# yuanhao-chen-nyoeghau/Wav2Vec2ForBrain

Measured on AMD Instinct MI355X. Metric: train steps/sec + CTC loss, b2p2t_gru+w2v bs=32 seq=1024, higher is better.
Workload: dtype bf16; 1 GPU; b2p2t_gru+w2v wav2vec2-base (12L/768), GRU H256x2 bidir, train mode, unfreeze=brain_encoder, Adam; global_batch=32, per_gpu_batch=32, seq_len=1024, parallelism=dp1

## Files before the change

### include/b2p_hip.h

```cpp
#ifndef B2P_HIP_H
#define B2P_HIP_H
#include <stdint.h>

#ifdef __cplusplus
extern "C" {
#endif

typedef void* b2p_stream_t;

const char* b2p_last_error(void);
int b2p_version(void);
int b2p_abi_sizes(int64_t* out3);
int b2p_timing_enable(int family, int max_events);
int b2p_timing_read(int family, float* total_ms, int* count, double* total_flops);

typedef struct {
  const void* ptr;
  int64_t ld;
  int64_t bs1, bs2;
  const int64_t* gather1;
  int32_t inner_is_k;
  int32_t conv;
  int32_t conv_T_out, conv_T_in, conv_stride, conv_pad, conv_Cg;
  int32_t dtype;
// ... 96 lines not shown
                      float* workspace, b2p_stream_t stream);
int b2p_layernorm_fwd16(const float* x, const float* gamma, const float* beta, float* y, uint16_t* y16,
                        float* mean, float* rstd, int64_t rows, int64_t cols, float eps,
                        float drop_p, uint64_t drop_seed, b2p_stream_t stream);
int b2p_layernorm_bwd16(const float* dy, const float* x, const float* gamma, const float* mean,
                        const float* rstd, float* dx, float* dgamma, float* dbeta, int64_t rows,
                        int64_t cols, const float* dx_accum, float drop_p, uint64_t drop_seed,
                        float* dx_dropped, float in_drop_p, uint64_t in_drop_seed, float* dbias_in,
                        uint16_t* d16, float* workspace, b2p_stream_t stream);
int b2p_layernorm_bwd_acc2(const float* dy, const float* x, const float* gamma, const float* mean,
                           const float* rstd, float* dx, float* dgamma, float* dbeta, int64_t rows,
                           int64_t cols, const float* dx_accum, const float* dx_accum2, float drop_p,
                           uint64_t drop_seed, float* dx_dropped, float in_drop_p, uint64_t in_drop_seed,
                           float* dbias_in, uint16_t* d16, float* workspace, b2p_stream_t stream);
int b2p_layernorm_fwd16_sel(const float* x, const float* gamma, const float* beta, float* y, uint16_t* y16,
                            float* mean, float* rstd, int64_t rows, int64_t cols, float eps, float drop_p,
                            uint64_t drop_seed, const int32_t* gate, const float* skip, const uint16_t* skip16,
                            b2p_stream_t stream);
int b2p_layernorm_fwd_x16_sel(const float* x, const float* gamma, const float* beta, float* y, uint16_t* y16,
                              int y16_fp16, uint16_t* y16b, float* mean, float* rstd, int64_t rows, int64_t cols,
                              float eps, const int32_t* gate, const float* skip, const uint16_t* skip16,
                              const uint16_t* skip16b, b2p_stream_t stream);
int b2p_layernorm_bwd_gated(const float* dy, const float* x, const float* gamma, const float* mean,
                            const float* rstd, float* dx, float* dgamma, float* dbeta, int64_t rows,
                            int64_t cols, const float* dx_accum, const float* dx_accum2, float drop_p,
                            uint64_t drop_seed, float* dx_dropped, float in_drop_p, uint64_t in_drop_seed,
                            float* dbias_in, uint16_t* d16, const int32_t* dy_gate, const int32_t* acc2_gate,
                            float* workspace, b2p_stream_t stream);
#define B2P_LNB_IN_DROP 1u
int b2p_layernorm_bwd_flags(const float* dy, const float* x, const float* gamma, const float* mean,
                            const float* rstd, float* dx, float* dgamma, float* dbeta, int64_t rows,
                            int64_t cols, const float* dx_accum, const float* dx_accum2, float drop_p,
                            uint64_t drop_seed, float* dx_dropped, float in_drop_p, uint64_t in_drop_seed,
                            float* dbias_in, uint16_t* d16, const int32_t* dy_gate, const int32_t* acc2_gate,
                            uint32_t flags, float* workspace, b2p_stream_t stream);

int b2p_cast_bf16(const float* x, uint16_t* y, int64_t n, b2p_stream_t stream);
int b2p_cast16_2d(const float* x, int64_t R, int64_t C, int64_t ldx, uint16_t* y, int64_t ldy, int fp16,
                  b2p_stream_t stream);
int b2p_transpose_bf16(const float* x, uint16_t* y, int64_t R, int64_t C, int64_t ldy, int64_t col0,
                       b2p_stream_t stream);

int b2p_softmax_fwd(const float* S, float* P, float* Pd, int64_t rows, int64_t n, int64_t ld,
                    float drop_p, uint64_t drop_seed, b2p_stream_t stream);
int b2p_softmax_bwd(const float* P, const float* dPd, float* dS, int64_t rows, int64_t n,
                    int64_t ld, float drop_p, uint64_t drop_seed, b2p_stream_t stream);

int b2p_act_fwd(const float* pre, float* out, int64_t n, int act, b2p_stream_t stream);
int b2p_act_bwd(const float* dy, const float* pre, float* dx, int64_t n, int act,
                b2p_stream_t stream);

int b2p_gauss_smooth(const float* x, const float* taps, int ntaps, float* y, int64_t B,
                     int64_t L, int64_t C, b2p_stream_t stream);
int b2p_unfold_col2im(const float* dA, const float* Z, float* dX, int64_t B, int64_t L,
                      int64_t C, int64_t T, int ktaps, int stride, b2p_stream_t stream);
int b2p_day_reduce(const float* per_sample, const int64_t* day_idx, int64_t B, int64_t ndays,
                   int64_t elems, float* out, b2p_stream_t stream);

int b2p_unfold16(const float* x, uint16_t* U, int64_t B, int64_t L, int64_t C, int64_t k,
                 int64_t stride, b2p_stream_t stream);
int b2p_unfold_weight16(const float* w0, const float* w1, int64_t G, int64_t C, int64_t k, int64_t stride,
                        uint16_t* wf, int fp16, uint16_t* wb, b2p_stream_t stream);
int b2p_pad_rows16(const float* src, uint16_t* dst, int64_t B, int64_t T, int64_t N, int64_t R, int64_t lead,
                   b2p_stream_t stream);
int b2p_cast16_tail(const float* x, uint16_t* y, int64_t n, int64_t n_total, int fp16, b2p_stream_t stream);
int b2p_gather_recs(const int64_t* recs, int nrec, b2p_stream_t stream);
int b2p_conv_weight_permute(const float* in, float* out, int64_t O, int64_t I, int64_t ntaps,
                            int inverse, b2p_stream_t stream);
int b2p_conv_weight_transpose_flip(const float* w, float* out, int64_t G, int64_t Og, int64_t I,
                                   int64_t ntaps, b2p_stream_t stream);

int b2p_ctc_greedy_wer(const float* logits, int64_t B, int64_t T, int64_t C, const int64_t* target, int64_t S,
                       int blank, int eos, int delim, int32_t* out_tokens, int32_t* out_ntok, int32_t* errs,
                       int32_t* nwords, b2p_stream_t stream);
int b2p_ctc_greedy_cer(const float* logits, int64_t B, int64_t T, int64_t C, const int64_t* target, int64_t S,
                       int blank, int eos, int delim, const uint8_t* tok_chars, const int32_t* tok_len,
                       int32_t* char_errs, int32_t* nchars, b2p_stream_t stream);
int64_t b2p_ctc_beam_workspace(int64_t B, int64_t T, int64_t beam);
int b2p_ctc_prefix_beam(const float* logits, int64_t B, int64_t T, int64_t C, const int32_t* lens, int64_t beam,
                        int blank, float token_min_logp, float beam_prune_logp, int32_t* workspace,
                        int32_t* out_tokens, int32_t* out_len, float* out_score, b2p_stream_t stream);
typedef struct {
  const uint64_t* trie_keys;
  const int32_t* trie_child;
  const int32_t* node_word;
  const uint64_t* ng_keys;
  const float* ng_vals;
  int64_t trie_capacity, ng_capacity;
  uint64_t trie_seed, ng_seed;
  int32_t order, unk_id, bos_id, eos_id;
  float beta;
  int32_t reserved;
} b2p_ngram_lm;
int64_t b2p_ctc_beam_lm_workspace(int64_t B, int64_t T, int64_t beam);
int b2p_ctc_prefix_beam_lm(const float* logits, int64_t B, int64_t T, int64_t C, const int32_t* lens, int64_t beam,
                           int blank, int delim, float token_min_logp, float beam_prune_logp,
                           const b2p_ngram_lm* lm, float unk_score_offset, float unk_score_scaled,
                           int score_boundary, int32_t* workspace, int32_t* out_tokens, int32_t* out_len,
                           float* out_ctc_logp, float* out_score, b2p_stream_t stream);

int b2p_posconv16_fwd(const float* e, const uint16_t* w16, const float* bias, float* xsum, float* pre,
                      uint16_t* e16, int64_t B, int64_t T, int64_t D, int64_t groups, b2p_stream_t stream);
int b2p_posconv16_bwd_data(const float* dxsum, const float* pre, const uint16_t* wt16, float* de, uint16_t* dpre16,
                           float* colpart, int64_t B, int64_t T, int64_t D, int64_t groups, b2p_stream_t stream);
int b2p_posconv16_wgrad(const uint16_t* dpre16, const uint16_t* e16, float* dwp, int64_t B, int64_t T, int64_t D,
                        int64_t groups, b2p_stream_t stream);
// ... 189 lines not shown
```

### wav2vec2forbrain_amd/_lib.py

```python
from __future__ import annotations

import ctypes
import os

import torch

_HERE = os.path.dirname(os.path.abspath(__file__))
LIB_PATH = os.environ.get("B2P_LIB_PATH") or os.path.join(_HERE, "libb2p_hip.so")

c_i64 = ctypes.c_int64
c_i32 = ctypes.c_int32
c_f32 = ctypes.c_float
c_f64 = ctypes.c_double
c_u64 = ctypes.c_uint64
c_u32 = ctypes.c_uint32
c_p = ctypes.c_void_p


class Operand(ctypes.Structure):
    _fields_ = [
        ("ptr", c_p), ("ld", c_i64), ("bs1", c_i64), ("bs2", c_i64), ("gather1", c_p),
        ("inner_is_k", c_i32), ("conv", c_i32),
        ("conv_T_out", c_i32), ("conv_T_in", c_i32), ("conv_stride", c_i32), ("conv_pad", c_i32),
        ("conv_Cg", c_i32), ("dtype", c_i32), ("conv_sample_stride", c_i64),
# ... 14 lines not shown
class GemmDesc(ctypes.Structure):
    _fields_ = [
        ("M", c_i64), ("N", c_i64), ("K", c_i64), ("nz1", c_i32), ("nz2", c_i32),
        ("A", Operand), ("B", Operand), ("ep", Epilogue),
        ("precision", c_i32), ("timing_family", c_i32), ("flops", c_f64),
        ("ksplit", c_i32), ("kchunk", c_i32), ("workspace", c_p), ("workspace_floats", c_i64),
    ]


class NgramLM(ctypes.Structure):
    _fields_ = [
        ("trie_keys", c_p), ("trie_child", c_p), ("node_word", c_p), ("ng_keys", c_p), ("ng_vals", c_p),
        ("trie_capacity", c_i64), ("ng_capacity", c_i64), ("trie_seed", c_u64), ("ng_seed", c_u64),
        ("order", c_i32), ("unk_id", c_i32), ("bos_id", c_i32), ("eos_id", c_i32), ("beta", c_f32),
        ("reserved", c_i32),
    ]


_SIGS = {
    "b2p_last_error": (ctypes.c_char_p, []),
    "b2p_version": (c_i32, []),
    "b2p_abi_sizes": (c_i32, [c_p]),
    "b2p_timing_enable": (c_i32, [c_i32, c_i32]),
    "b2p_timing_read": (c_i32, [c_i32, ctypes.POINTER(c_f32), ctypes.POINTER(c_i32), ctypes.POINTER(c_f64)]),
    "b2p_gemm": (c_i32, [ctypes.POINTER(GemmDesc), c_p]),
    "b2p_colsum_workspace": (c_i64, [c_i64, c_i64]),
    "b2p_colsum": (c_i32, [c_p, c_i64, c_i64, c_i64, c_p, c_i32, c_p, c_p]),
    "b2p_colsum_batched": (c_i32, [c_p, c_p, c_i64, c_i64, c_i64, c_i64, c_i64, c_i32, c_p, c_i32, c_p, c_p]),
    "b2p_colsum_parts": (c_i32, [c_p, c_i64, c_i64, c_p, c_i32, c_p]),
    "b2p_attn16_dkv_variant": (c_i32, [c_i32]),
    "b2p_set_gate_batch": (c_i32, [c_p]),
    "b2p_split3_bf16": (c_i32, [c_p, c_i64, c_i64, c_i64, c_p, c_i64, c_i32, c_i32, c_p]),
    "b2p_i64_fill": (c_i32, [c_p, ctypes.POINTER(c_i64), c_i32, c_p]),
    "b2p_colsum_pin_begin": (c_i32, []),
    "b2p_colsum_pin_end": (c_i64, []),
    "b2p_colsum_unpin": (c_i32, [c_i64]),
    "b2p_colsum_pool_state": (c_i64, [c_i64, ctypes.POINTER(c_i64)]),
    "b2p_dropout": (c_i32, [c_p, c_p, c_i64, c_f32, c_u64, c_p]),
    "b2p_layernorm_fwd": (c_i32, [c_p, c_p, c_p, c_p, c_p, c_p, c_i64, c_i64, c_f32, c_f32, c_u64, c_p]),
    "b2p_layernorm_bwd_workspace": (c_i64, [c_i64, c_i64]),
    "b2p_layernorm_bwd": (c_i32, [c_p, c_p, c_p, c_p, c_p, c_p, c_p, c_p, c_i64, c_i64, c_p, c_f32, c_u64,
                                  c_p, c_f32, c_u64, c_p, c_p, c_p]),
    "b2p_layernorm_fwd16": (c_i32, [c_p, c_p, c_p, c_p, c_p, c_p, c_p, c_i64, c_i64, c_f32, c_f32, c_u64, c_p]),
    "b2p_layernorm_bwd16": (c_i32, [c_p, c_p, c_p, c_p, c_p, c_p, c_p, c_p, c_i64, c_i64, c_p, c_f32, c_u64,
                                    c_p, c_f32, c_u64, c_p, c_p, c_p, c_p]),
    "b2p_layernorm_bwd_acc2": (c_i32, [c_p, c_p, c_p, c_p, c_p, c_p, c_p, c_p, c_i64, c_i64, c_p, c_p, c_f32, c_u64,
                                       c_p, c_f32, c_u64, c_p, c_p, c_p, c_p]),
    "b2p_cast_bf16": (c_i32, [c_p, c_p, c_i64, c_p]),
    "b2p_softmax_fwd": (c_i32, [c_p, c_p, c_p, c_i64, c_i64, c_i64, c_f32, c_u64, c_p]),
    "b2p_softmax_bwd": (c_i32, [c_p, c_p, c_p, c_i64, c_i64, c_i64, c_f32, c_u64, c_p]),
    "b2p_act_fwd": (c_i32, [c_p, c_p, c_i64, c_i32, c_p]),
    "b2p_act_bwd": (c_i32, [c_p, c_p, c_p, c_i64, c_i32, c_p]),
    "b2p_gauss_smooth": (c_i32, [c_p, c_p, c_i32, c_p, c_i64, c_i64, c_i64, c_p]),
    "b2p_unfold_col2im": (c_i32, [c_p, c_p, c_p, c_i64, c_i64, c_i64, c_i64, c_i32, c_i32, c_p]),
    "b2p_day_reduce": (c_i32, [c_p, c_p, c_i64, c_i64, c_i64, c_p, c_p]),
    "b2p_unfold16": (c_i32, [c_p, c_p, c_i64, c_i64, c_i64, c_i64, c_i64, c_p]),
    "b2p_unfold_weight16": (c_i32, [c_p, c_p, c_i64, c_i64, c_i64, c_i64, c_p, c_i32, c_p, c_p]),
    "b2p_pad_rows16": (c_i32, [c_p, c_p, c_i64, c_i64, c_i64, c_i64, c_i64, c_p]),
    "b2p_cast16_tail": (c_i32, [c_p, c_p, c_i64, c_i64, c_i32, c_p]),
    "b2p_gather_recs": (c_i32, [c_p, c_i32, c_p]),
    "b2p_conv_weight_permute": (c_i32, [c_p, c_p, c_i64, c_i64, c_i64, c_i32, c_p]),
    "b2p_conv_weight_transpose_flip": (c_i32, [c_p, c_p, c_i64, c_i64, c_i64, c_i64, c_p]),
    "b2p_weight_norm_workspace": (c_i64, [c_i64, c_i64, c_i64]),
    "b2p_weight_norm_fwd": (c_i32, [c_p, c_p, c_p, c_p, c_i64, c_i64, c_i64, c_p, c_p]),
    "b2p_weight_norm_bwd": (c_i32, [c_p, c_p, c_p, c_p, c_p, c_p, c_i64, c_i64, c_i64, c_p, c_p]),
    "b2p_gru_fwd": (c_i32, [c_p, c_p, c_p, c_p, c_p, c_p, c_i64, c_i64, c_i64, c_i32, c_p]),
    "b2p_gru_bwd": (c_i32, [c_p, c_p, c_p, c_p, c_p, c_p, c_p, c_p, c_p, c_i64, c_i64, c_i64, c_i32, c_p]),
    "b2p_gru16_supported": (c_i32, [c_i64]),
    "b2p_gru16_lane_floats": (c_i64, [c_i64, c_i64, c_i64, c_i32, c_i32]),
    "b2p_gru_lane_permute": (c_i32, [c_p, c_p, c_i64, c_i64, c_i64, c_i32, c_i32, c_i32, c_u32, c_i32, c_p]),
    "b2p_gru_fwd16": (c_i32, [c_p, c_p, c_p, c_p, c_p, c_p, c_i64, c_i64, c_i64, c_i32, c_p]),
    "b2p_gru_bwd16": (c_i32, [c_p, c_p, c_p, c_p, c_p, c_p, c_p, c_i64, c_i64, c_i64, c_i32, c_p]),
    "b2p_gru_mc_supported": (c_i32, [c_i64]),
    "b2p_gru_mc_workspace": (c_i64, [c_i64, c_i64, c_i32]),
    "b2p_gru_fwd_mc": (c_i32, [c_p, c_p, c_p, c_p, c_p, c_p, c_p, c_i64, c_i64, c_i64, c_i32, c_p]),
    "b2p_gru_bwd_mc": (c_i32, [c_p, c_p, c_p, c_p, c_p, c_p, c_p, c_p, c_p, c_i64, c_i64, c_i64, c_i32, c_p]),
    "b2p_gru_mc_status": (c_i32, [c_p, c_p, c_i32, c_p]),
    "b2p_gru_mc_debug_withhold": (c_i32, [c_i32]),
    "b2p_gru32_supported": (c_i32, [c_i64]),
    "b2p_gru32_workspace": (c_i64, [c_i64, c_i64, c_i32]),
    "b2p_gru_fwd32": (c_i32, [c_p, c_p, c_p, c_p, c_p, c_p, c_p, c_i64, c_i64, c_i64, c_i32, c_p]),
    "b2p_gru_bwd32": (c_i32, [c_p, c_p, c_p, c_p, c_p, c_p, c_p, c_p, c_p, c_i64, c_i64, c_i64, c_i32, c_p]),
    "b2p_gru_hprev": (c_i32, [c_p, c_p, c_p, c_i64, c_i64, c_i64, c_i32, c_p]),
    "b2p_attn16_fwd": (c_i32, [c_p, c_p, c_p, c_i64, c_i64, c_i64, c_i64, c_f32, c_f32, c_u64, c_p, c_p]),
    "b2p_attn16_fwd_f16": (c_i32, [c_p, c_p, c_p, c_p, c_i64, c_i64, c_i64, c_i64, c_f32, c_f32, c_u64, c_p, c_p]),
    "b2p_attn16_fwd_keep": (c_i32, [c_p, c_p, c_p, c_i64, c_i64, c_i64, c_i64, c_f32, c_f32, c_p, c_p]),
    "b2p_attn16_fwd_f16_keep": (c_i32, [c_p, c_p, c_p, c_p, c_i64, c_i64, c_i64, c_i64, c_f32, c_f32, c_p, c_p]),
    "b2p_attn16_keep_masks": (c_i32, [c_p, c_p, c_i64, c_i64, c_i64, c_i64, c_f32, c_p]),
    "b2p_attn16_bwd": (c_i32, [c_p, c_p, c_p, c_p, c_p, c_p, c_i64, c_i64, c_i64, c_i64, c_f32, c_f32, c_u64, c_p,
                               c_p]),
    "b2p_attn16_bwd_f16": (c_i32, [c_p, c_p, c_p, c_p, c_p, c_p, c_i64, c_i64, c_i64, c_i64, c_f32, c_f32, c_u64, c_p,
                               c_p]),
    "b2p_attn32_supported": (c_i32, [c_i64, c_i64]),
    "b2p_attn32_fwd": (c_i32, [c_p, c_p, c_p, c_i64, c_i64, c_i64, c_i64, c_f32, c_f32, c_u64, c_p]),
    "b2p_attn32_bwd": (c_i32, [c_p, c_p, c_p, c_p, c_p, c_i64, c_i64, c_i64, c_i64, c_f32, c_f32, c_u64, c_p]),
    "b2p_attn32_long_supported": (c_i32, [c_i64, c_i64]),
    "b2p_attn32_long_fwd": (c_i32, [c_p, c_p, c_p, c_i64, c_i64, c_i64, c_i64, c_f32, c_f32, c_u64, c_p]),
    "b2p_attn32_long_bwd": (c_i32, [c_p, c_p, c_p, c_p, c_p, c_i64, c_i64, c_i64, c_i64, c_f32, c_f32, c_u64, c_p]),
    "b2p_ctc_workspace": (c_i64, [c_i64, c_i64, c_i64, c_i64]),
    "b2p_ctc_fwd_bwd": (c_i32, [c_p, c_p, c_p, c_p, c_i64, c_i64, c_i64, c_i64, c_i32, c_p, c_p, c_p, c_p, c_p]),
    "b2p_adam_multi": (c_i32, [c_p, c_i32, c_i64, c_f32, c_f32, c_f32, c_f32, c_f32, c_f32, c_f32, c_p]),
    "b2p_adam_multi_dev": (c_i32, [c_p, c_i32, c_i64, c_p, c_f32, c_f32, c_f32, c_f32, c_p, c_p, c_p]),
    "b2p_cast16_2d": (c_i32, [c_p, c_i64, c_i64, c_i64, c_p, c_i64, c_i32, c_p]),
    "b2p_accum_recs": (c_i32, [c_p, c_i32, c_p]),
    "b2p_accum_rows_recs": (c_i32, [c_p, c_i32, c_p]),
    "b2p_adam_recs": (c_i32, [c_p, c_i32, c_f32, c_f64, c_f64, c_f32, c_f32, c_f32, c_f32, c_p, c_p, c_p, c_p]),
# ... 114 lines not shown
```

### wav2vec2forbrain_amd/functional.py

```python
from __future__ import annotations

import collections
import contextlib
import functools
import ctypes
import math
import threading
import weakref

import os

import torch

from . import _lib
from ._lib import GemmDesc, Operand, Epilogue

ACT = {"none": 0, None: 0, "gelu": 1, "softsign": 2, "silu": 3, "swish": 3,
       "linear": 0, "gelu_python": 1,
       "gelu_new": 4, "gelu_fast": 4, "gelu_pytorch_tanh": 4, "gelu_accurate": 4,
       "gelu_10": 5, "quick_gelu": 6, "laplace": 7, "mish": 8, "relu": 9, "relu2": 10, "relu6": 11,
       "sigmoid": 12, "tanh": 13}
EPILOGUE_ACTS = frozenset({0, 1, 2, 3})
_ACT_NAME = {}
for _k, _v in ACT.items():
# ... 1174 lines not shown
def to16h(x):
    t = getattr(x, "_h16", None)
    if t is not None and t[0] == x._version:
        return t[1]
    xc = x.contiguous()
    out = torch.empty(xc.shape, device=x.device, dtype=torch.float16)
    _lib.call("b2p_cast16_2d", _p(xc), 1, xc.numel(), xc.numel(), _p(out), xc.numel(), 1, _st())
    return out


def _ln_fwd16(x2d, g, b, eps, drop_p=0.0, seed=0, sel=None):
    rows, cols = x2d.shape
    y = torch.empty_like(x2d)
    y16 = torch.empty(rows, cols, device=x2d.device, dtype=BF16)
    mean = torch.empty(rows, device=x2d.device)
    rstd = torch.empty(rows, device=x2d.device)
    if sel is not None:
        _lib.call("b2p_layernorm_fwd16_sel", _p(x2d), _p(g), _p(b), _p(y), _p(y16), _p(mean), _p(rstd), rows, cols,
                  float(eps), float(drop_p), seed, _p(sel[0]), _p(sel[1]), _p(sel[2]), _st())
        return y, y16, mean, rstd
    _lib.call("b2p_layernorm_fwd16", _p(x2d), _p(g), _p(b), _p(y), _p(y16), _p(mean), _p(rstd), rows, cols,
              float(eps), float(drop_p), seed, _st())
    return y, y16, mean, rstd


def _ln_bwd16(dy, x, g, mean, rstd, need_params=True, dx_accum=None, drop_p=0.0, seed=0, in_drop_p=-1.0,
              in_seed=0, dbias_in=None, dx_accum2=None, lazy=None, dy_gate=None, acc2_gate=None, want_dxd=True):
    rows, cols = x.shape
    lz = _ln_lazy(lazy, need_params, dbias_in)
    dx = torch.empty_like(x)
    dg = torch.empty(cols, device=x.device) if need_params and not lz else None
    db = torch.empty(cols, device=x.device) if need_params and not lz else None
    ws = torch.empty(int(_lib.load().b2p_layernorm_bwd_workspace(rows, cols)), device=x.device)
    dxd = torch.empty_like(x) if in_drop_p >= 0.0 and want_dxd else None
    d16 = torch.empty(rows, cols, device=x.device, dtype=BF16)
    if in_drop_p >= 0.0 and not want_dxd:
        _lib.call("b2p_layernorm_bwd_flags", _p(dy), _p(x), _p(g), _p(mean), _p(rstd), _p(dx), _p(dg), _p(db), rows,
                  cols, _p(dx_accum), _p(dx_accum2), float(drop_p), seed, None, float(in_drop_p), in_seed,
                  None if lz else _p(dbias_in), _p(d16), _p(dy_gate), _p(acc2_gate), _lib.LNB_IN_DROP, _p(ws), _st())
    elif dy_gate is not None or acc2_gate is not None:
        _lib.call("b2p_layernorm_bwd_gated", _p(dy), _p(x), _p(g), _p(mean), _p(rstd), _p(dx), _p(dg), _p(db), rows,
                  cols, _p(dx_accum), _p(dx_accum2), float(drop_p), seed, _p(dxd), float(max(in_drop_p, 0.0)),
                  in_seed, None if lz else _p(dbias_in), _p(d16), _p(dy_gate), _p(acc2_gate), _p(ws), _st())
    else:
        _lib.call("b2p_layernorm_bwd_acc2", _p(dy), _p(x), _p(g), _p(mean), _p(rstd), _p(dx), _p(dg), _p(db), rows,
                  cols, _p(dx_accum), _p(dx_accum2), float(drop_p), seed, _p(dxd), float(max(in_drop_p, 0.0)),
                  in_seed, None if lz else _p(dbias_in), _p(d16), _p(ws), _st())
    if lz:
        dg, db = _ln_parts(ws, rows, cols, 0), _ln_parts(ws, rows, cols, 1)
        dbias_in = _ln_parts(ws, rows, cols, 2) if dbias_in is not None else None
    return (dx, dg, db, dxd, d16) if lazy is None else (dx, dg, db, dxd, d16, dbias_in)


@_prec_follow
class _FrontEnd(torch.autograd.Function):
    @staticmethod
    def forward(ctx, x, day_idxs, day_weights, day_bias, taps):
        _chk(x, "front_end.x")
        _chk(day_weights, "front_end.day_weights")
        B, L, C = x.shape
        xs = torch.empty_like(x)
        _lib.call("b2p_gauss_smooth", _p(x), _p(taps), taps.numel(), _p(xs), B, L, C, _st())
        z = torch.empty_like(x)
        s = torch.empty_like(x)
        gemm(L, C, C, op(xs, 0, C, True, bs1=L * C), op(day_weights, 0, C, False, bs1=C * C, gather=day_idxs),
             s, C, cbs1=L * C, nz1=B, bias=day_bias, biasbs1=C, bias_gather=day_idxs, pre_out=z,
             act=ACT["softsign"])
        ctx.save_for_backward(xs, z, day_idxs, day_weights)
        ctx.n_days = day_weights.shape[0]
        return s

    @staticmethod
    def backward(ctx, ds):
        xs, z, day_idxs, day_weights = ctx.saved_tensors
        ds = ds.contiguous()
        B, L, C = xs.shape
        dz = _act_bwd(ds, z, ACT["softsign"])
        dW = dbias = None
        if ctx.needs_input_grad[2]:
            per = torch.empty(B, C, C, device=xs.device)
            gemm(C, C, L, op(xs, 0, C, False, bs1=L * C), op(dz, 0, C, False, bs1=L * C), per, C, cbs1=C * C, nz1=B)
            dW = torch.empty_like(day_weights)
            _lib.call("b2p_day_reduce", _p(per), _p(day_idxs), B, ctx.n_days, C * C, _p(dW), _st())
        if ctx.needs_input_grad[3]:
            per_b = torch.empty(B, C, device=xs.device)
            colsum_batched(dz, B, L, C, per_b)
            dbias = torch.empty(ctx.n_days, 1, C, device=xs.device)
            _lib.call("b2p_day_reduce", _p(per_b), _p(day_idxs), B, ctx.n_days, C, _p(dbias), _st())
        return None, None, dW, dbias, None


def front_end(x, day_idxs, day_weights, day_bias, taps):
    with _fp32_if("front"):
        return _FrontEnd.apply(x.contiguous(), day_idxs.to(torch.int64).contiguous(), day_weights, day_bias, taps)


class Unfolded:

    def __init__(self, src: torch.Tensor, kernel: int, stride: int):
        self.src = src
        self.kernel = kernel
        self.stride = stride
        B, L, C = src.shape
        self.T = (L - kernel) // stride + 1
        self.shape = (B, self.T, C * kernel)

    def materialize(self) -> torch.Tensor:
        B, L, C = self.src.shape
        idx = torch.arange(self.T, device=self.src.device)[:, None] * self.stride + torch.arange(self.kernel, device=self.src.device)[None, :]
        win = self.src[:, idx, :]
        return win.permute(0, 1, 3, 2).reshape(B, self.T, C * self.kernel)


_GRUMC = [True]
_GRUMC_BWD = [None]
_GRU32 = [True]
GRU32_MODES = (3,)
_GRU32_NARROW_MAX = 512


@contextlib.contextmanager
def persistent_gru32(on: bool = True):
    old = _GRU32[0]
    _GRU32[0] = bool(on)
    try:
        yield
    finally:
        _GRU32[0] = old


def _gru_recurrence(H: int) -> str:
    lib = _lib.load()
    fast = bf16_mode() or (_state.prec == 3 and "grurec1" in (_state.x3forms or ()))
    if fast and lib.b2p_gru16_supported(H):
        return "gru16"
    if fast and _GRUMC[0] and lib.b2p_gru_mc_supported(H):
        return "mc"
    if not fast and _state.prec in GRU32_MODES and _GRU32[0] and lib.b2p_gru32_supported(H):
        if H <= _GRU32_NARROW_MAX or "gru32w" in (_state.x3forms or ()):
            return "gru32"
    return "step"


def _gru_recurrence_bwd(fwd: str, H: int) -> str:
    if fwd == "gru16" or _GRUMC_BWD[0] is None:
        return fwd
    if _GRUMC_BWD[0] and _lib.load().b2p_gru_mc_supported(H):
# ... 132 lines not shown

class _UnfoldProj:

    @staticmethod
    def forward(x, wih, bias_cat, gi, s, need_dx):
        B, T, IN, G3, N3, L, C = s.B, s.T, s.IN, s.G3, s.N3, s.L, s.C
        wperm = torch.empty(N3, IN, device=s.dev)
        for d in range(s.ndir):
            _lib.call("b2p_conv_weight_permute", _p(wih[d]), _p(wperm, d * G3 * IN), G3, C, s.ktaps, 0, _st())
        U16 = None
        if bf16_mode() and not _state.fwd16:
            U16 = torch.empty(B * T, IN, device=s.dev, dtype=BF16)
            _lib.call("b2p_unfold16", _p(x), _p(U16), B, L, C, s.ktaps, s.stride, _st())
            wperm = cast16(wperm)
            A = op(U16, 0, IN, True)
        else:
            A = conv_op(x, 0, C, T, L, s.stride, 0, IN, L * C, True)
            A.conv_Cg = C
        gemm(B * T, N3, IN, A, op(wperm, 0, IN, True), gi, N3, bias=bias_cat)
        return wperm, U16

    @staticmethod
    def backward(dgi, x, wih, kept, s, need_dx, need_dw):
        B, T, IN, N3, L, C = s.B, s.T, s.IN, s.N3, s.L, s.C
        wperm, U16 = kept
        dg = cast16(dgi) if U16 is not None else dgi
        dx, dws = None, [None] * s.ndir
        if any(need_dw):
            dwp = torch.empty(N3, IN, device=s.dev)
            U = op(U16, 0, IN, False) if U16 is not None else conv_op(x, 0, C, T, L, s.stride, 0, C, L * C, False)
            gemm(N3, IN, B * T, op(dg, 0, N3, False), U, dwp, IN)
            dws = _unfold_dw(dwp, s)
        if need_dx:
            dA = torch.empty(B * T, IN, device=s.dev)
            gemm(B * T, IN, N3, op(dg, 0, N3, True), op(wperm, 0, IN, False), dA, IN)
            dx = torch.empty(B, L, C, device=s.dev)
            _lib.call("b2p_unfold_col2im", _p(dA), None, _p(dx), B, L, C, T, s.ktaps, s.stride, _st())
        return dx, dws


class _ImplicitUnfoldProj:

    @staticmethod
    def forward(x, wih, bias_cat, gi, s, need_dx):
        B, T, IN, N3, L, C, ktaps, stride = s.B, s.T, s.IN, s.N3, s.L, s.C, s.ktaps, s.stride
        half = _state.fwd16
        wf = torch.empty(N3, IN, device=s.dev, dtype=torch.float16 if half else BF16)
        wperm = torch.empty((ktaps // stride) * N3, stride * C, device=s.dev, dtype=BF16) if need_dx else None
        _lib.call("b2p_unfold_weight16", _p(wih[0]), _p(wih[1]) if s.ndir == 2 else None, s.G3, C, ktaps, stride,
                  _p(wf), int(half), _p(wperm), _st())
        s16 = _ImplicitUnfoldProj.source16(x, s, half)
        gemm(T, N3, IN, op(s16, 0, stride * C, True, bs1=L * C), op(wf, 0, IN, True), gi, N3, cbs1=T * N3, nz1=B,
             bias=bias_cat)
        return wperm, (None if half else s16)

    @staticmethod
    def source16(x, s, half):
        n_s, tail = s.B * s.L * s.C, (s.ktaps - s.stride) * s.C
        s16 = torch.empty(n_s + tail, device=s.dev, dtype=torch.float16 if half else BF16)
        _lib.call("b2p_cast16_tail", _p(x), _p(s16), n_s, n_s + tail, int(half), _st())
        return s16

    @staticmethod
    def backward(dgi, x, wih, kept, s, need_dx, need_dw):
        B, IN, N3, L, C, ktaps, stride = s.B, s.IN, s.N3, s.L, s.C, s.ktaps, s.stride
        wperm, s16 = kept
        R, lead = L // stride, ktaps // stride - 1
        dgp = torch.empty((lead + B * R) * N3, device=s.dev, dtype=BF16)
        _lib.call("b2p_pad_rows16", _p(dgi), _p(dgp), B, s.T, N3, R, lead, _st())
        dx, dws = None, [None] * s.ndir
        if any(need_dw):
            s16 = s16 if s16 is not None else _ImplicitUnfoldProj.source16(x, s, False)
            dwp = torch.empty(N3, IN, device=s.dev)
            gemm(N3, IN, B * R, op(dgp, lead * N3, N3, False), op(s16, 0, stride * C, False), dwp, IN)
            del s16
            dws = _unfold_dw(dwp, s)
        if need_dx:
            dx = torch.empty(B, L, C, device=s.dev)
            gemm(B * R, stride * C, (ktaps // stride) * N3, op(dgp, 0, N3, True), op(wperm, 0, stride * C, False),
                 dx, stride * C)
        return dx, dws


@_prec_follow
class _GRULayer(torch.autograd.Function):
    @staticmethod
    def forward(ctx, x, unf_meta, H, ndir, h0, *weights):
        dev, G3 = x.device, 3 * H
        if unf_meta is not None:
            ktaps, stride = unf_meta
            B, L, C = x.shape
            s = _GRUShape(B, (L - ktaps) // stride + 1, C * ktaps, H, G3, ndir * G3, ndir, dev, L, C, ktaps, stride)
        else:
            s = _GRUShape(*x.shape, H, G3, ndir * G3, ndir, dev, None, None, None, None)
        B, T = s.B, s.T
        wih, whh, bih, bhh = ([weights[4 * d + i] for d in range(ndir)] for i in range(4))
        for w in wih + whh:
            _chk(w, "gru.weight")
        gi = torch.empty(B, T, ndir * G3, device=dev)
        rec = _gru_recurrence(H)
        fold = rec == "gru16" and bhh[0] is not None
        whh_s = torch.empty(ndir, G3, H, device=dev)
        bhh_s = torch.empty(ndir, G3, device=dev) if bhh[0] is not None else None
        bias_cat = torch.empty(ndir * G3, device=dev) if (any(b is not None for b in bih) or fold) else None
        recs = []
        for d in range(ndir):
            recs += [_p(whh_s, d * G3 * H), _p(whh[d]), 0, G3 * H]
            if bhh_s is not None:
                recs += [_p(bhh_s, d * G3), _p(bhh[d]), 0, G3]
            if bias_cat is not None:
# ... 1811 lines not shown
```

### wav2vec2forbrain_amd/model/b2p2t_model.py

```python
from __future__ import annotations

import math
from typing import Literal, cast

import torch
from pydantic import BaseModel
from torch import nn

from .. import functional as Fn
from ..datasets.batch_types import B2tSampleBatch
from .b2tmodel import B2TModel, ModelOutput

DEFAULT_UNFOLDER_KERNEL_LEN = 32


class B2P2TModelArgsModel(BaseModel):
    input_layer_nonlinearity: Literal["softsign"] = "softsign"
    unfolder_kernel_len: int = DEFAULT_UNFOLDER_KERNEL_LEN
    unfolder_stride_len: int = 4
    gaussian_smooth_width: float = 0.3


class GaussianSmoothing(nn.Module):

    def __init__(self, channels, kernel_size: int, sigma: float, dim=1):
        super().__init__()
        if dim != 1:
            raise NotImplementedError("only the 1-D smoothing used by B2P2TModel is supported")
        mgrid = torch.arange(kernel_size, dtype=torch.float32)
        mean = (kernel_size - 1) / 2
        kernel = 1 / (sigma * math.sqrt(2 * math.pi)) * torch.exp(-(((mgrid - mean) / sigma) ** 2) / 2)
        kernel = kernel / torch.sum(kernel)
        kernel = kernel.view(1, 1, kernel_size).repeat(channels, 1, 1)
        self.register_buffer("weight", kernel)
        self.groups = channels

    def taps(self) -> torch.Tensor:
        return self.weight[0, 0].contiguous()


class B2P2TModel(B2TModel):

    def __init__(self, config: B2P2TModelArgsModel, neural_decoder: B2TModel, pad_token_id=0):
        super().__init__()
        self.config = config
        self.pad_token_id = pad_token_id
        if config.input_layer_nonlinearity != "softsign":
            raise NotImplementedError("Only softsign is currently supported as input layer nonlinearity")
        n_days = 24
        neural_dim_len = 256
        self.gaussian_smoother = GaussianSmoothing(neural_dim_len, 20, config.gaussian_smooth_width, dim=1)
        self.day_weights = nn.Parameter(torch.randn(n_days, neural_dim_len, neural_dim_len))
        self.day_bias = nn.Parameter(torch.zeros(n_days, 1, neural_dim_len))
        for x in range(n_days):
            self.day_weights.data[x, :, :] = torch.eye(neural_dim_len)
        self.neural_decoder = neural_decoder
        for x in range(n_days):
            setattr(self, "inpLayer" + str(x), nn.Linear(neural_dim_len, neural_dim_len))
        for x in range(n_days):
            layer = getattr(self, "inpLayer" + str(x))
            layer.weight = nn.Parameter(layer.weight + torch.eye(neural_dim_len))

    def forward(self, batch: B2tSampleBatch) -> ModelOutput:
        x, targets = batch
        day_idxs = batch.day_idxs
        taps = self.gaussian_smoother.taps()
        s = Fn.front_end(x, day_idxs, self.day_weights, self.day_bias, taps)
        strided_inputs = Fn.Unfolded(s, self.config.unfolder_kernel_len, self.config.unfolder_stride_len)
        preprocessed_batch = batch.copy_and_change(input=strided_inputs)
        if hasattr(batch, "input_lens"):
            processed_in_lens = Fn.unfold_lens(batch.input_lens, self.config.unfolder_kernel_len,
                                               self.config.unfolder_stride_len)
            preprocessed_batch.input_lens = processed_in_lens
            out = self.neural_decoder.forward(preprocessed_batch)
            out.logit_lens = processed_in_lens
            return out
        return self.neural_decoder.forward(preprocessed_batch)

    def output_length(self, L: int) -> int:
        return (L - self.config.unfolder_kernel_len) // self.config.unfolder_stride_len + 1

    @classmethod
    def get_in_size_after_preprocessing(cls, unfolder_kernel_len: int):
        return 256 * unfolder_kernel_len
```

Before: 78.84 steps/s.

## Fuse front-end gaussian smoothing, day GEMM and softsign into one MFMA kernel

```diff
diff --git a/include/b2p_hip.h b/include/b2p_hip.h
--- a/include/b2p_hip.h
+++ b/include/b2p_hip.h
@@ -172,6 +172,14 @@
 
 int b2p_gauss_smooth(const float* x, const float* taps, int ntaps, float* y, int64_t B,
                      int64_t L, int64_t C, b2p_stream_t stream);
+int b2p_front16_supported(int64_t C, int ntaps);
+int b2p_front16_fwd(const float* x, const float* taps, int ntaps, const int64_t* day_idx, const float* day_w,
+                    const float* day_b, int64_t ndays, float* z, float* s, uint16_t* s_f16, uint16_t* s_bf16,
+                    uint16_t* xs_bf16, int64_t B, int64_t L, int64_t C, int64_t tail, int fp16,
+                    b2p_stream_t stream);
+int64_t b2p_front16_bwd_workspace(int64_t B, int64_t L, int64_t C);
+int b2p_front16_bwd(const float* ds, const float* z, uint16_t* dz_bf16, const int64_t* day_idx, int64_t ndays,
+                    float* dbias, int64_t B, int64_t L, int64_t C, float* workspace, b2p_stream_t stream);
 int b2p_unfold_col2im(const float* dA, const float* Z, float* dX, int64_t B, int64_t L,
                       int64_t C, int64_t T, int ktaps, int stride, b2p_stream_t stream);
 int b2p_day_reduce(const float* per_sample, const int64_t* day_idx, int64_t B, int64_t ndays,
diff --git a/wav2vec2forbrain_amd/_lib.py b/wav2vec2forbrain_amd/_lib.py
--- a/wav2vec2forbrain_amd/_lib.py
+++ b/wav2vec2forbrain_amd/_lib.py
@@ -90,6 +90,11 @@
     "b2p_act_fwd": (c_i32, [c_p, c_p, c_i64, c_i32, c_p]),
     "b2p_act_bwd": (c_i32, [c_p, c_p, c_p, c_i64, c_i32, c_p]),
     "b2p_gauss_smooth": (c_i32, [c_p, c_p, c_i32, c_p, c_i64, c_i64, c_i64, c_p]),
+    "b2p_front16_supported": (c_i32, [c_i64, c_i32]),
+    "b2p_front16_fwd": (c_i32, [c_p, c_p, c_i32, c_p, c_p, c_p, c_i64, c_p, c_p, c_p, c_p, c_p, c_i64, c_i64, c_i64,
+                                c_i64, c_i32, c_p]),
+    "b2p_front16_bwd_workspace": (c_i64, [c_i64, c_i64, c_i64]),
+    "b2p_front16_bwd": (c_i32, [c_p, c_p, c_p, c_p, c_i64, c_p, c_i64, c_i64, c_i64, c_p, c_p]),
     "b2p_unfold_col2im": (c_i32, [c_p, c_p, c_p, c_i64, c_i64, c_i64, c_i64, c_i32, c_i32, c_p]),
     "b2p_day_reduce": (c_i32, [c_p, c_p, c_i64, c_i64, c_i64, c_p, c_p]),
     "b2p_unfold16": (c_i32, [c_p, c_p, c_i64, c_i64, c_i64, c_i64, c_i64, c_p]),
diff --git a/wav2vec2forbrain_amd/csrc/front16.hip b/wav2vec2forbrain_amd/csrc/front16.hip
--- /dev/null
+++ b/wav2vec2forbrain_amd/csrc/front16.hip
@@ -0,0 +1,256 @@
+#include "common.h"
+#include "act.h"
+#include "../../include/b2p_hip.h"
+
+namespace {
+constexpr int F16_C = 256;
+constexpr int F16_TM = 64;
+constexpr int F16_LDA = F16_C + 8;
+constexpr int F16_KT = 32;
+constexpr int F16_LDW = F16_KT + 8;
+constexpr int F16_LDS_STAGE = 132;
+constexpr int F16_MAXTAPS = 64;
+
+template <bool HALF> __device__ __forceinline__ uint2 f16_pack4(float4 v) {
+  return HALF ? b2p_pack_f16x4(v) : b2p_pack_bf16x4(v);
+}
+template <bool HALF> __device__ __forceinline__ f32x4 f16_mfma(const bf16x8& a, const bf16x8& b, const f32x4& c) {
+  if constexpr (HALF) return b2p_mfma_f16(a, b, c);
+  else return __builtin_amdgcn_mfma_f32_16x16x32_bf16(a, b, c, 0, 0, 0);
+}
+
+template <bool HALF>
+__global__ void __launch_bounds__(256) front16_fwd_k(const float* __restrict__ x, const float* __restrict__ taps,
+                                                     int ntaps, const int64_t* __restrict__ day,
+                                                     const float* __restrict__ W, const float* __restrict__ bias,
+                                                     float* __restrict__ z, float* __restrict__ s,
+                                                     uint16_t* __restrict__ sh, uint16_t* __restrict__ sb,
+                                                     uint16_t* __restrict__ xs16, int64_t B, int64_t L,
+                                                     int64_t tail4) {
+  __shared__ __attribute__((aligned(16))) uint16_t As[F16_TM * F16_LDA];
+  __shared__ __attribute__((aligned(16))) uint16_t Ws[F16_C * F16_LDW];
+  __shared__ float tapz[F16_MAXTAPS + 40];
+  const int tid = threadIdx.x, lane = tid & 63, w = tid >> 6;
+  const int64_t b = blockIdx.y, l0 = (int64_t)blockIdx.x * F16_TM;
+  const int64_t d = day[b];
+
+  if (blockIdx.x == gridDim.x - 1 && b == B - 1)
+    for (int64_t i = tid; i < tail4; i += 256) {
+      if (sh) reinterpret_cast<uint2*>(sh)[B * L * (F16_C / 4) + i] = make_uint2(0u, 0u);
+      if (sb) reinterpret_cast<uint2*>(sb)[B * L * (F16_C / 4) + i] = make_uint2(0u, 0u);
+    }
+
+  for (int i = tid; i < F16_MAXTAPS + 40; i += 256) tapz[i] = (i >= 16 && i < 16 + ntaps) ? taps[i - 16] : 0.f;
+
+  const float* Wd = W + d * (int64_t)(F16_C * F16_C);
+  const int kb = lane >> 4, n4 = 16 * w + (lane & 15);
+  float4 wr[8];
+#pragma unroll
+  for (int kk = 0; kk < 8; ++kk)
+    wr[kk] = *reinterpret_cast<const float4*>(Wd + (int64_t)(8 * kb + kk) * F16_C + 4 * n4);
+  __syncthreads();
+
+  {
+    const int left = (ntaps - 1) / 2;
+    const int64_t rbase = l0 + 16 * w;
+    const float4* xb = reinterpret_cast<const float4*>(x) + b * L * (F16_C / 4) + lane;
+    float4 acc[16];
+#pragma unroll
+    for (int r = 0; r < 16; ++r) acc[r] = make_float4(0.f, 0.f, 0.f, 0.f);
+    const int T = 16 + ntaps - 1;
+    auto load4 = [&](float4 (&v)[4], int t0) {
+#pragma unroll
+      for (int q = 0; q < 4; ++q) {
+        const int64_t src = rbase - left + t0 + q;
+        const bool in = src >= 0 && src < L && t0 + q < T;
+        const float4 u = xb[(in ? src : 0) * (F16_C / 4)];
+        v[q] = in ? u : make_float4(0.f, 0.f, 0.f, 0.f);
+      }
+    };
+    float4 nv[4];
+    load4(nv, 0);
+    for (int t0 = 0; t0 < T; t0 += 4) {
+      float4 v[4];
+#pragma unroll
+      for (int q = 0; q < 4; ++q) v[q] = nv[q];
+      if (t0 + 4 < T) load4(nv, t0 + 4);
+#pragma unroll
+      for (int q = 0; q < 4; ++q)
+#pragma unroll
+        for (int r = 0; r < 16; ++r) {
+          const float wt = tapz[16 + t0 + q - r];
+          acc[r].x += wt * v[q].x; acc[r].y += wt * v[q].y; acc[r].z += wt * v[q].z; acc[r].w += wt * v[q].w;
+        }
+    }
+#pragma unroll
+    for (int r = 0; r < 16; ++r) {
+      const uint2 pb = b2p_pack_bf16x4(acc[r]);
+      if (rbase + r < L) reinterpret_cast<uint2*>(xs16)[(b * L + rbase + r) * (F16_C / 4) + lane] = pb;
+      *reinterpret_cast<uint2*>(&As[(16 * w + r) * F16_LDA + 4 * lane]) = HALF ? b2p_pack_f16x4(acc[r]) : pb;
+    }
+  }
+  __syncthreads();
+  bf16x8 xf[8];
+#pragma unroll
+  for (int ks = 0; ks < 8; ++ks)
+    xf[ks] = *reinterpret_cast<const bf16x8*>(&As[(16 * w + (lane & 15)) * F16_LDA + 32 * ks + 8 * kb]);
+
+  f32x4 acc[16];
+#pragma unroll
+  for (int nt = 0; nt < 16; ++nt) acc[nt] = f32x4{0.f, 0.f, 0.f, 0.f};
+#pragma unroll
+  for (int kt = 0; kt < F16_C / F16_KT; ++kt) {
+    if (kt) __syncthreads();
+#pragma unroll
+    for (int i = 0; i < 4; ++i) {
+      float c[8];
+#pragma unroll
+      for (int kk = 0; kk < 8; ++kk) c[kk] = i == 0 ? wr[kk].x : i == 1 ? wr[kk].y : i == 2 ? wr[kk].z : wr[kk].w;
+      uint4 p;
+      const uint2 lo = f16_pack4<HALF>(make_float4(c[0], c[1], c[2], c[3]));
+      const uint2 hi = f16_pack4<HALF>(make_float4(c[4], c[5], c[6], c[7]));
+      p.x = lo.x; p.y = lo.y; p.z = hi.x; p.w = hi.y;
+      *reinterpret_cast<uint4*>(&Ws[(4 * n4 + i) * F16_LDW + 8 * kb]) = p;
+    }
+    __syncthreads();
+    if (kt + 1 < F16_C / F16_KT) {
+#pragma unroll
+      for (int kk = 0; kk < 8; ++kk)
+        wr[kk] = *reinterpret_cast<const float4*>(Wd + (int64_t)(F16_KT * (kt + 1) + 8 * kb + kk) * F16_C + 4 * n4);
+    }
+#pragma unroll
+    for (int nt = 0; nt < 16; ++nt) {
+      const bf16x8 wf = *reinterpret_cast<const bf16x8*>(&Ws[(16 * nt + (lane & 15)) * F16_LDW + 8 * kb]);
+      acc[nt] = f16_mfma<HALF>(wf, xf[kt], acc[nt]);
+    }
+  }
+
+  float* stage = reinterpret_cast<float*>(&As[16 * w * F16_LDA]);
+  const float* bd = bias + d * F16_C;
+  const int c4 = lane & 31, rh = lane >> 5;
+#pragma unroll
+  for (int h = 0; h < 2; ++h) {
+    __syncthreads();
+#pragma unroll
+    for (int nt = 0; nt < 8; ++nt)
+      *reinterpret_cast<f32x4*>(&stage[(lane & 15) * F16_LDS_STAGE + 16 * nt + 4 * kb]) = acc[8 * h + nt];
+    __syncthreads();
+    const float4 bv = *reinterpret_cast<const float4*>(bd + 128 * h + 4 * c4);
+#pragma unroll
+    for (int rr = 0; rr < 8; ++rr) {
+      const int r = 2 * rr + rh;
+      const int64_t row = l0 + 16 * w + r;
+      if (row >= L) continue;
+      float4 zv = *reinterpret_cast<const float4*>(&stage[r * F16_LDS_STAGE + 4 * c4]);
+      zv.x += bv.x; zv.y += bv.y; zv.z += bv.z; zv.w += bv.w;
+      const float4 sv = make_float4(b2p_act_val<B2P_ACT_SOFTSIGN>(zv.x), b2p_act_val<B2P_ACT_SOFTSIGN>(zv.y),
+                                    b2p_act_val<B2P_ACT_SOFTSIGN>(zv.z), b2p_act_val<B2P_ACT_SOFTSIGN>(zv.w));
+      const int64_t o = (b * L + row) * (F16_C / 4) + 32 * h + c4;
+      reinterpret_cast<float4*>(z)[o] = zv;
+      reinterpret_cast<float4*>(s)[o] = sv;
+      if (sh) reinterpret_cast<uint2*>(sh)[o] = b2p_pack_f16x4(sv);
+      if (sb) reinterpret_cast<uint2*>(sb)[o] = b2p_pack_bf16x4(sv);
+    }
+  }
+}
+
+constexpr int F16_BR = 32;
+
+__global__ void __launch_bounds__(256) front16_bwd_k(const float4* __restrict__ ds, const float4* __restrict__ z,
+                                                     uint2* __restrict__ dz16, float* __restrict__ part,
+                                                     int64_t L) {
+  __shared__ float4 red[4][64];
+  const int c4 = threadIdx.x & 63, rl = threadIdx.x >> 6;
+  const int64_t b = blockIdx.y, r0 = (int64_t)blockIdx.x * F16_BR;
+  const int64_t r1 = r0 + F16_BR < L ? r0 + F16_BR : L;
+  float4 sum = make_float4(0.f, 0.f, 0.f, 0.f);
+#pragma unroll 4
+  for (int64_t r = r0 + rl; r < r1; r += 4) {
+    const int64_t o = (b * L + r) * (F16_C / 4) + c4;
+    const float4 g = ds[o], p = z[o];
+    const float4 v = make_float4(g.x * b2p_act_grad<B2P_ACT_SOFTSIGN>(p.x), g.y * b2p_act_grad<B2P_ACT_SOFTSIGN>(p.y),
+                                 g.z * b2p_act_grad<B2P_ACT_SOFTSIGN>(p.z), g.w * b2p_act_grad<B2P_ACT_SOFTSIGN>(p.w));
+    dz16[o] = b2p_pack_bf16x4(v);
+    sum.x += v.x; sum.y += v.y; sum.z += v.z; sum.w += v.w;
+  }
+  red[rl][c4] = sum;
+  __syncthreads();
+  if (rl == 0) {
+    float4 t = red[0][c4];
+#pragma unroll
+    for (int i = 1; i < 4; ++i) {
+      const float4 u = red[i][c4];
+      t.x += u.x; t.y += u.y; t.z += u.z; t.w += u.w;
+    }
+    reinterpret_cast<float4*>(part)[(b * gridDim.x + blockIdx.x) * (F16_C / 4) + c4] = t;
+  }
+}
+
+__global__ void front16_bias_k(const float* __restrict__ part, const int64_t* __restrict__ day, int64_t B,
+                               int64_t ndays, int nblk, float* __restrict__ dbias) {
+  const int64_t i = (int64_t)blockIdx.x * blockDim.x + threadIdx.x;
+  if (i >= ndays * F16_C) return;
+  const int64_t d = i / F16_C, c = i % F16_C;
+  float acc = 0.f;
+  for (int64_t b = 0; b < B; ++b) {
+    if (day[b] != d) continue;
+    float sb = 0.f;
+    for (int k = 0; k < nblk; ++k) sb += part[(b * nblk + k) * F16_C + c];
+    acc += sb;
+  }
+  dbias[i] = acc;
+}
+
+inline bool a16(const void* p) { return ((uintptr_t)p & 15u) == 0; }
+}
+
+extern "C" int b2p_front16_supported(int64_t C, int ntaps) {
+  return C == F16_C && ntaps > 0 && ntaps <= F16_MAXTAPS;
+}
+
+extern "C" int b2p_front16_fwd(const float* x, const float* taps, int ntaps, const int64_t* day_idx,
+                               const float* day_w, const float* day_b, int64_t ndays, float* z, float* s,
+                               uint16_t* s_f16, uint16_t* s_bf16, uint16_t* xs_bf16, int64_t B, int64_t L,
+                               int64_t C, int64_t tail, int fp16, b2p_stream_t stream) {
+  B2P_CHECK_ARG(x && taps && day_idx && day_w && day_b && z && s && xs_bf16, "front16_fwd: NULL pointer");
+  B2P_CHECK_ARG(b2p_front16_supported(C, ntaps), "front16_fwd: needs C == 256 and 1 <= ntaps <= 64 (C %lld, ntaps %d)",
+                (long long)C, ntaps);
+  B2P_CHECK_ARG(ndays > 0 && tail >= 0 && tail % 4 == 0, "front16_fwd: bad ndays / tail");
+  B2P_CHECK_ARG(a16(x) && a16(day_w) && a16(day_b) && a16(z) && a16(s) && a16(s_f16) && a16(s_bf16) && a16(xs_bf16),
+                "front16_fwd: pointers must be 16-byte aligned");
+  B2P_CHECK_ARG(B < 65536 && L < (1ll << 31), "front16_fwd: B or L too large");
+  if (B <= 0 || L <= 0) return 0;
+  const dim3 grid((unsigned)((L + F16_TM - 1) / F16_TM), (unsigned)B);
+  if (fp16)
+    hipLaunchKernelGGL(front16_fwd_k<true>, grid, dim3(256), 0, (hipStream_t)stream, x, taps, ntaps, day_idx, day_w,
+                       day_b, z, s, s_f16, s_bf16, xs_bf16, B, L, tail / 4);
+  else
+    hipLaunchKernelGGL(front16_fwd_k<false>, grid, dim3(256), 0, (hipStream_t)stream, x, taps, ntaps, day_idx, day_w,
+                       day_b, z, s, s_f16, s_bf16, xs_bf16, B, L, tail / 4);
+  B2P_CHECK_LAUNCH();
+  return 0;
+}
+
+extern "C" int64_t b2p_front16_bwd_workspace(int64_t B, int64_t L, int64_t C) {
+  return B * ((L + F16_BR - 1) / F16_BR) * C;
+}
+
+extern "C" int b2p_front16_bwd(const float* ds, const float* z, uint16_t* dz_bf16, const int64_t* day_idx,
+                               int64_t ndays, float* dbias, int64_t B, int64_t L, int64_t C, float* workspace,
+                               b2p_stream_t stream) {
+  B2P_CHECK_ARG(ds && z && dz_bf16 && workspace, "front16_bwd: NULL pointer");
+  B2P_CHECK_ARG(C == F16_C, "front16_bwd: needs C == 256 (C %lld)", (long long)C);
+  B2P_CHECK_ARG(!dbias || (day_idx && ndays > 0), "front16_bwd: dbias needs day_idx and ndays");
+  B2P_CHECK_ARG(a16(ds) && a16(z) && a16(dz_bf16) && a16(workspace), "front16_bwd: pointers must be 16-byte aligned");
+  B2P_CHECK_ARG(B < 65536 && L < (1ll << 31), "front16_bwd: B or L too large");
+  if (B <= 0 || L <= 0) return 0;
+  const int nblk = (int)((L + F16_BR - 1) / F16_BR);
+  hipLaunchKernelGGL(front16_bwd_k, dim3((unsigned)nblk, (unsigned)B), dim3(256), 0, (hipStream_t)stream,
+                     reinterpret_cast<const float4*>(ds), reinterpret_cast<const float4*>(z),
+                     reinterpret_cast<uint2*>(dz_bf16), workspace, L);
+  if (dbias)
+    hipLaunchKernelGGL(front16_bias_k, dim3((unsigned)((ndays * F16_C + 255) / 256)), dim3(256), 0, (hipStream_t)stream,
+                       workspace, day_idx, B, ndays, nblk, dbias);
+  B2P_CHECK_LAUNCH();
+  return 0;
+}
diff --git a/wav2vec2forbrain_amd/functional.py b/wav2vec2forbrain_amd/functional.py
--- a/wav2vec2forbrain_amd/functional.py
+++ b/wav2vec2forbrain_amd/functional.py
@@ -1250,13 +1250,50 @@
     return (dx, dg, db, dxd, d16) if lazy is None else (dx, dg, db, dxd, d16, dbias_in)
 
 
+_FRONT16 = [True]
+
+
+@contextlib.contextmanager
+def fused_front16(on: bool = True):
+    old = _FRONT16[0]
+    _FRONT16[0] = bool(on)
+    try:
+        yield
+    finally:
+        _FRONT16[0] = old
+
+
+def _front16_ok(x, day_weights, day_bias, taps) -> bool:
+    C = x.shape[-1]
+    return (_FRONT16[0] and bf16_mode() and "bwd32path" not in DIAG_SWITCHES and day_bias is not None
+            and tuple(day_weights.shape[1:]) == (C, C) and day_bias.is_contiguous() and day_bias.dtype == torch.float32
+            and bool(_lib.load().b2p_front16_supported(C, taps.numel()))
+            and all(t.data_ptr() % 16 == 0 for t in (x, day_weights, day_bias)))
+
+
 @_prec_follow
 class _FrontEnd(torch.autograd.Function):
     @staticmethod
-    def forward(ctx, x, day_idxs, day_weights, day_bias, taps):
+    def forward(ctx, x, day_idxs, day_weights, day_bias, taps, tail_rows=0):
         _chk(x, "front_end.x")
         _chk(day_weights, "front_end.day_weights")
         B, L, C = x.shape
+        ctx.fused = _front16_ok(x, day_weights, day_bias, taps)
+        ctx.n_days = day_weights.shape[0]
+        if ctx.fused:
+            half = _state.fwd16
+            n_s, tail = B * L * C, max(int(tail_rows), 0) * C
+            z, s = torch.empty_like(x), torch.empty_like(x)
+            sh = torch.empty(n_s + tail, device=x.device, dtype=torch.float16) if half else None
+            sb = torch.empty(n_s + tail, device=x.device, dtype=BF16)
+            xs16 = torch.empty(B, L, C, device=x.device, dtype=BF16)
+            _lib.call("b2p_front16_fwd", _p(x), _p(taps), taps.numel(), _p(day_idxs), _p(day_weights), _p(day_bias),
+                      ctx.n_days, _p(z), _p(s), _p(sh), _p(sb), _p(xs16), B, L, C, tail, int(half), _st())
+            ctx.save_for_backward(xs16, z, day_idxs)
+            attach16(s, sb)
+            if half:
+                attach16h(s, sh)
+            return s
         xs = torch.empty_like(x)
         _lib.call("b2p_gauss_smooth", _p(x), _p(taps), taps.numel(), _p(xs), B, L, C, _st())
         z = torch.empty_like(x)
@@ -1265,13 +1302,39 @@
              s, C, cbs1=L * C, nz1=B, bias=day_bias, biasbs1=C, bias_gather=day_idxs, pre_out=z,
              act=ACT["softsign"])
         ctx.save_for_backward(xs, z, day_idxs, day_weights)
-        ctx.n_days = day_weights.shape[0]
         return s
 
     @staticmethod
+    def _backward16(ctx, ds):
+        xs16, z, day_idxs = ctx.saved_tensors
+        B, L, C = xs16.shape
+        dev = xs16.device
+        dW = dbias = None
+        if not (ctx.needs_input_grad[2] or ctx.needs_input_grad[3]):
+            return None, None, None, None, None, None
+        if ds.data_ptr() % 16:
+            ds = ds.clone()
+        dz16 = torch.empty(B, L, C, device=dev, dtype=BF16)
+        ws = torch.empty(int(_lib.load().b2p_front16_bwd_workspace(B, L, C)), device=dev)
+        if ctx.needs_input_grad[3]:
+            dbias = torch.empty(ctx.n_days, 1, C, device=dev)
+        _lib.call("b2p_front16_bwd", _p(ds), _p(z), _p(dz16), _p(day_idxs), ctx.n_days, _p(dbias), B, L, C, _p(ws),
+                  _st())
+        if ctx.needs_input_grad[2]:
+            per = torch.empty(B, C, C, device=dev)
+            with precision("bf16"):
+                gemm(C, C, L, op(xs16, 0, C, False, bs1=L * C), op(dz16, 0, C, False, bs1=L * C), per, C,
+                     cbs1=C * C, nz1=B)
+            dW = torch.empty(ctx.n_days, C, C, device=dev)
+            _lib.call("b2p_day_reduce", _p(per), _p(day_idxs), B, ctx.n_days, C * C, _p(dW), _st())
+        return None, None, dW, dbias, None, None
+
+    @staticmethod
     def backward(ctx, ds):
+        ds = ds.contiguous()
+        if ctx.fused:
+            return _FrontEnd._backward16(ctx, ds)
         xs, z, day_idxs, day_weights = ctx.saved_tensors
-        ds = ds.contiguous()
         B, L, C = xs.shape
         dz = _act_bwd(ds, z, ACT["softsign"])
         dW = dbias = None
@@ -1285,12 +1348,13 @@
             colsum_batched(dz, B, L, C, per_b)
             dbias = torch.empty(ctx.n_days, 1, C, device=xs.device)
             _lib.call("b2p_day_reduce", _p(per_b), _p(day_idxs), B, ctx.n_days, C, _p(dbias), _st())
-        return None, None, dW, dbias, None
-
-
-def front_end(x, day_idxs, day_weights, day_bias, taps):
+        return None, None, dW, dbias, None, None
+
+
+def front_end(x, day_idxs, day_weights, day_bias, taps, tail_rows=0):
     with _fp32_if("front"):
-        return _FrontEnd.apply(x.contiguous(), day_idxs.to(torch.int64).contiguous(), day_weights, day_bias, taps)
+        return _FrontEnd.apply(x.contiguous(), day_idxs.to(torch.int64).contiguous(), day_weights, day_bias, taps,
+                               tail_rows)
 
 
 class Unfolded:
@@ -1529,10 +1593,19 @@
         s16 = _ImplicitUnfoldProj.source16(x, s, half)
         gemm(T, N3, IN, op(s16, 0, stride * C, True, bs1=L * C), op(wf, 0, IN, True), gi, N3, cbs1=T * N3, nz1=B,
              bias=bias_cat)
-        return wperm, (None if half else s16)
+        return wperm, (_ImplicitUnfoldProj.tagged16(x, s, False) if half else s16)
+
+    @staticmethod
+    def tagged16(x, s, half):
+        t = _h16_of(x) if half else _b16_of(x)
+        need = s.B * s.L * s.C + (s.ktaps - s.stride) * s.C
+        return t if t is not None and t.dim() == 1 and t.numel() >= need else None
 
     @staticmethod
     def source16(x, s, half):
+        t = _ImplicitUnfoldProj.tagged16(x, s, half)
+        if t is not None:
+            return t
         n_s, tail = s.B * s.L * s.C, (s.ktaps - s.stride) * s.C
         s16 = torch.empty(n_s + tail, device=s.dev, dtype=torch.float16 if half else BF16)
         _lib.call("b2p_cast16_tail", _p(x), _p(s16), n_s, n_s + tail, int(half), _st())
diff --git a/wav2vec2forbrain_amd/model/b2p2t_model.py b/wav2vec2forbrain_amd/model/b2p2t_model.py
--- a/wav2vec2forbrain_amd/model/b2p2t_model.py
+++ b/wav2vec2forbrain_amd/model/b2p2t_model.py
@@ -65,7 +65,8 @@
         x, targets = batch
         day_idxs = batch.day_idxs
         taps = self.gaussian_smoother.taps()
-        s = Fn.front_end(x, day_idxs, self.day_weights, self.day_bias, taps)
+        s = Fn.front_end(x, day_idxs, self.day_weights, self.day_bias, taps,
+                         tail_rows=self.config.unfolder_kernel_len - self.config.unfolder_stride_len)
         strided_inputs = Fn.Unfolded(s, self.config.unfolder_kernel_len, self.config.unfolder_stride_len)
         preprocessed_batch = batch.copy_and_change(input=strided_inputs)
         if hasattr(batch, "input_lens"):
```

Result: no change. 79.54 steps/s, median of 6 (+0.9%).
